# RoboticExplorationLab/TrajectoryOptimization.jl

Hardware: NVIDIA H100
Metric: ilqr_iterations_per_sec (higher is better)
Workload: dtype f64

## Files before the change

### profiles/linesearch_ab.py

```python
#!/usr/bin/env python3
import argparse, json, os, subprocess, sys, tempfile

import numpy as np

ROOT = os.path.dirname(os.path.dirname(os.path.abspath(__file__)))
DEFAULT = os.path.join(ROOT, "trajectoryoptimization.jl_b200", "libtrajopt_b200.so")
VARIANT = os.path.join(ROOT, "trajectoryoptimization.jl_b200", "variants", "lib_fwd_loop.so")


def card():
    q = subprocess.run(["nvidia-smi", "--query-gpu=name,power.limit,clocks.max.sm", "--format=csv,noheader"], capture_output=True, text=True)
    return q.stdout.strip().splitlines()[0] if q.returncode == 0 and q.stdout.strip() else "unknown"


def bench(lib, workload, dump):
    env = dict(os.environ, LIBTRAJOPT_B200=lib)
    out = subprocess.run([sys.executable, os.path.join(ROOT, "bench.py"), "--gpus", "1", "--steps", "20", "--warmup", "3", "--workload", workload,
                          "--no-cpu-baseline", "--dump-outputs", dump], capture_output=True, text=True, env=env, cwd=ROOT)
    line = [l for l in out.stdout.splitlines() if l.startswith("{")]
    if out.returncode or not line:
        raise SystemExit(f"bench.py failed on {lib}:\n{out.stderr[-2000:]}")
    d = json.loads(line[-1])
    ph = d["roofline"]["phase_ms"]
    return dict(step=d["ms_per_step"], F=ph["forward"], L=ph["ladder"], C1E1=ph["cost_expansion"] + ph["expand"],
                E2C2=ph["late_expansion"], R=ph["backward"], phases=ph)


def main():
    ap = argparse.ArgumentParser()
    ap.add_argument("--reps", type=int, default=3)
    ap.add_argument("--workload", default="quadrotor")
    ap.add_argument("--out", default=None)
    ap.add_argument("--lib", action="append", default=[], metavar="NAME=PATH", help="further libraries to alternate with the two")
    args = ap.parse_args()
    tmp = tempfile.mkdtemp(prefix="linesearch_ab_")
    variant = VARIANT
    if not os.path.exists(variant):
        subprocess.run(["bash", os.path.join(ROOT, "profiles", "scripts", "build_variant.sh"), "fwd_loop", "forward.cu", "-DTO_FWD_COMPACT=0"],
                       check=True, env=dict(os.environ, VARIANT_DIR=tmp), stdout=subprocess.DEVNULL)
        variant = os.path.join(tmp, "lib_fwd_loop.so")
    print(f"card: {card()}  workload: {args.workload}", flush=True)
    libs = {"rollout_fast (-DTO_FWD_COMPACT=0)": variant, "rollout_compact (default)": DEFAULT}
    libs.update(dict(kv.split("=", 1) for kv in args.lib))
    runs = {name: [] for name in libs}
    dumps = []
    for r in range(args.reps):
        for name, lib in libs.items():
            d = os.path.join(tmp, f"dump_{len(dumps)}")
            res = bench(lib, args.workload, d)
            runs[name].append(res); dumps.append((name, d))
            print(f"  {name:36s} step {res['step']:.4f}  F {res['F']:.4f}  L {res['L']:.4f}  C1+E1 {res['C1E1']:.4f}  "
                  f"E2/C2 {res['E2C2']:.4f}  R {res['R']:.4f}", flush=True)
    ref_name, ref = dumps[0]
    identical = True
    for name, d in dumps[1:]:
        for f in sorted(os.listdir(ref)):
            a, b = np.load(os.path.join(ref, f)), np.load(os.path.join(d, f))
            if a.shape != b.shape or not np.array_equal(a.view(np.uint8), b.view(np.uint8)):
                identical = False
                print(f"  DUMP DIFFERS: {f} of {name} against {ref_name}")
    print(f"dumps bit-identical across all {len(dumps)} runs: {identical}")
    for name, rs in runs.items():
        rng = lambda k: f"{min(x[k] for x in rs):.3f}-{max(x[k] for x in rs):.3f}"
        print(f"{name:36s} step {rng('step')}  F {rng('F')}  L {rng('L')}  C1+E1 {rng('C1E1')}  E2/C2 {rng('E2C2')}  R {rng('R')}")
    fa, fb = runs["rollout_fast (-DTO_FWD_COMPACT=0)"], runs["rollout_compact (default)"]
    print(f"every default run faster than every variant run: {max(x['step'] for x in fb) < min(x['step'] for x in fa)}")
    if args.out:
        with open(args.out, "w") as fh:
            json.dump(dict(card=card(), runs=runs, identical=identical), fh, indent=1)
    sys.exit(0 if identical else 1)


if __name__ == "__main__":
    main()
```

### trajectoryoptimization.jl_b200/csrc/capi.cu

```cuda
#include <cmath>
#include <cstdio>
#include <cstring>
#include <string>
#include <vector>

#include "../../include/trajopt_b200.h"
#include "frag_layout.cuh"
#include "kernels.h"

namespace {

std::string g_create_error;

struct Scratch {
    void* ptr = nullptr;
    size_t bytes = 0;
};

}

struct to_handle {
    DevProblem P{};
    int device = 0;
    cudaStream_t stream = nullptr;
// ... 559 lines not shown
        P.max_cons_knot = std::max(P.max_cons_knot, nk);
    }
    {
        bool cls = N >= 2 && P.all_diag_cost && P.all_diag_con;
        for (int k = 1; k < N - 1; k++) if (h->h_cost_index[k] != h->h_cost_index[0]) cls = false;
        int nbox = 0, ngc = 0;
        for (const auto& c : h->h_cons) {
            if (c.kind == CON_BOUND) {
                bool ubox = c.first == 1 && c.last == N - 1 && c.p == 2 * m;
                for (int j = 0; j < n + m; j++) if ((c.row_max[j] >= 0) != (j >= n) || (c.row_min[j] >= 0) != (j >= n)) ubox = false;
                cls = cls && ubox; nbox++;
            } else if (c.kind == CON_GOAL) {
                cls = cls && c.first == N && c.last == N; ngc++;
            } else cls = false;
        }
        P.fwd_compact = (cls && nbox <= 1 && ngc <= 1) ? 1 : 0;
    }
    h->h_mu.assign(s->ncon, P.opt.penalty_initial);
    h->h_dt.assign(s->dt, s->dt + (N - 1));
    h->h_dyn = dyn_tab; h->h_dyn_index = dyn_idx;

    int rc = TO_OK;
    double* d_dt = nullptr; int* d_ci = nullptr;
    P.strideX = (size_t)B * N * n; P.strideU = (size_t)B * (N - 1) * m;
#define ALLOC(ptr, count) if (!rc) rc = dalloc(h, &(ptr), (size_t)(count))
    ALLOC(d_dt, N - 1); ALLOC(d_ci, N);
    DevDyn* d_dyn = nullptr; int* d_dyni = nullptr;
    if (!h->h_dyn.empty()) { ALLOC(d_dyn, h->h_dyn.size()); ALLOC(d_dyni, N - 1); }
    ALLOC(h->d_costs, s->ncost); ALLOC(h->d_cons, std::max(1, s->ncon)); ALLOC(h->d_mu, std::max(1, s->ncon));
    ALLOC(P.x0, (size_t)B * n); ALLOC(P.X, TO_NBUF * P.strideX); ALLOC(P.U, TO_NBUF * P.strideU); ALLOC(P.cur, B);
    ALLOC(P.AB, (size_t)B * (N - 1) * n * P.ldab); ALLOC(P.K, (size_t)B * (N - 1) * P.ne * m); ALLOC(P.d, (size_t)B * (N - 1) * m);
    if (P.dense_riccati) {
        const size_t nme = P.ne + m;
        ALLOC(P.ABe, (size_t)B * (N - 1) * P.ne * nme); ALLOC(P.EG, (size_t)B * N * nme); ALLOC(P.EH, (size_t)B * N * nme * nme);
        if (P.compact) ALLOC(P.EC, (size_t)B * N * TO_EC_LEN);
        if (P.frag) ALLOC(P.REC, (size_t)B * N * TO_REC_LEN);
    }
    ALLOC(P.lambda, (size_t)B * std::max(1, P.lambda_len));
    ALLOC(P.rho, B); ALLOC(P.drho, B); ALLOC(P.dV, 2 * (size_t)B); ALLOC(P.J, B); ALLOC(P.Jc, B); ALLOC(P.alpha, B);
    ALLOC(P.bp_status, B); ALLOC(P.ls_iters, B); ALLOC(P.accepted, B); ALLOC(P.acc1, B);
    if (P.frag) { ALLOC(P.late_list, B); ALLOC(P.late_count, 1); }
    ALLOC(h->d_stageX, P.strideX); ALLOC(h->d_stageU, P.strideU); ALLOC(h->d_viol, B); ALLOC(h->d_merit2, 2);
    ALLOC(h->d_work, 1); ALLOC(h->d_err, 1);
    {
        SolveDev& S = h->solve;
        ALLOC(S.state, B); ALLOC(S.status, B); ALLOC(S.iter, B); ALLOC(S.outer, B); ALLOC(S.inner, B); ALLOC(S.dj_zero, B);
        ALLOC(S.J_prev, B); ALLOC(S.dJ, B); ALLOC(S.grad, B); ALLOC(S.cmax, B); ALLOC(S.n_active, 1);
    }
    if (P.frag) { ALLOC(h->d_fragq, frag_queue_ints(B)); ALLOC(h->d_fragpool, frag_pool_doubles(B, N)); ALLOC(h->d_fragerr, 1); ALLOC(h->d_exptab, 1); }
#undef ALLOC
    if (rc) return bail(rc);
    P.exptab = h->d_exptab;
    P.dyn = d_dyn; P.dyn_index = d_dyni;
    P.dt = d_dt; P.cost_index = d_ci; P.costs = h->d_costs; P.cons = h->d_cons; P.mu = h->d_mu; P.viol = h->d_viol;
    cudaStream_t st = h->stream;
    bool okc = true;
    okc &= cudaMemcpyAsync(d_dt, h->h_dt.data(), sizeof(double) * (N - 1), cudaMemcpyHostToDevice, st) == cudaSuccess;
    okc &= cudaMemcpyAsync(d_ci, h->h_cost_index.data(), sizeof(int) * N, cudaMemcpyHostToDevice, st) == cudaSuccess;
    if (d_dyn) {
        okc &= cudaMemcpyAsync(d_dyn, h->h_dyn.data(), sizeof(DevDyn) * h->h_dyn.size(), cudaMemcpyHostToDevice, st) == cudaSuccess;
        okc &= cudaMemcpyAsync(d_dyni, h->h_dyn_index.data(), sizeof(int) * (N - 1), cudaMemcpyHostToDevice, st) == cudaSuccess;
    }
    okc &= cudaMemsetAsync(P.x0, 0, sizeof(double) * B * n, st) == cudaSuccess;
    okc &= cudaMemsetAsync(P.X, 0xFF, sizeof(double) * TO_NBUF * P.strideX, st) == cudaSuccess;
    okc &= cudaMemsetAsync(P.U, 0, sizeof(double) * TO_NBUF * P.strideU, st) == cudaSuccess;
// ... 123 lines not shown
        if (upper) upper[i] = up;
    }
    return TO_OK;
}

int to_set_initial_state(to_handle* h, const double* x0) {
    JOIN(h);
    if (!h || !x0) return TO_EINVAL;
    CU(h, cudaMemcpyAsync(h->P.x0, x0, sizeof(double) * (size_t)h->P.B * h->P.n, cudaMemcpyHostToDevice, h->stream));
    h->J_valid = false;
    return TO_OK;
}
int to_set_controls(to_handle* h, const double* U) {
    JOIN(h);
    if (!h || !U) return TO_EINVAL;
    CU(h, cudaMemcpyAsync(h->d_stageU, U, sizeof(double) * h->P.strideU, cudaMemcpyHostToDevice, h->stream));
    CU(h, launch_scatter_traj(h->P, nullptr, h->d_stageU, h->stream)); h->launches++;
    h->J_valid = false; h->expanded = false; h->backward_done = false;
    return TO_OK;
}
int to_set_states(to_handle* h, const double* X) {
    JOIN(h);
    if (!h || !X) return TO_EINVAL;
    CU(h, cudaMemcpyAsync(h->d_stageX, X, sizeof(double) * h->P.strideX, cudaMemcpyHostToDevice, h->stream));
    CU(h, launch_scatter_traj(h->P, h->d_stageX, nullptr, h->stream)); h->launches++;
    h->J_valid = false; h->expanded = false; h->backward_done = false;
    return TO_OK;
}
int to_get_states(to_handle* h, double* X) {
    JOIN(h);
    if (!h || !X) return TO_EINVAL;
    CU(h, launch_gather_traj(h->P, h->d_stageX, nullptr, h->stream)); h->launches++;
    CU(h, cudaMemcpyAsync(X, h->d_stageX, sizeof(double) * h->P.strideX, cudaMemcpyDeviceToHost, h->stream));
    CU(h, cudaStreamSynchronize(h->stream));
    return TO_OK;
}
int to_get_controls(to_handle* h, double* U) {
    JOIN(h);
    if (!h || !U) return TO_EINVAL;
    CU(h, launch_gather_traj(h->P, nullptr, h->d_stageU, h->stream)); h->launches++;
    CU(h, cudaMemcpyAsync(U, h->d_stageU, sizeof(double) * h->P.strideU, cudaMemcpyDeviceToHost, h->stream));
    CU(h, cudaStreamSynchronize(h->stream));
    return TO_OK;
}
int to_get_times(to_handle* h, double* t) {
    JOIN(h);
    if (!h || !t) return TO_EINVAL;
    t[0] = h->t0;
    for (int k = 1; k < h->P.N; k++) t[k] = t[k - 1] + h->h_dt[k - 1];
    return TO_OK;
}
int to_set_initial_time(to_handle* h, double t0, double* tf_out) {
    JOIN(h);
    if (!h) return TO_EINVAL;
    h->t0 = t0;
    if (tf_out) { double t = t0; for (double d : h->h_dt) t += d; *tf_out = t; }
// ... 855 lines not shown
```

### trajectoryoptimization.jl_b200/csrc/common.cuh

```cuda
#pragma once
#include <cuda_runtime.h>
#include <cstdlib>
#include <stdint.h>

#define TO_MAXN 16
#define TO_MAXM 8
#define TO_MAXNM (TO_MAXN + TO_MAXM)
#define TO_MAXCON 8
#define TO_MAXP 32
#define TO_MAXPV (2 * TO_MAXNM)
#define TO_CON_A 256
#define TO_EXPR_LEN 128
#define TO_EXPR_CONST 64
#define TO_EC_LEN 40
#define TO_NBUF 9

enum { MODEL_DOUBLE_INTEGRATOR = 0, MODEL_CARTPOLE = 1, MODEL_QUADROTOR = 2, MODEL_ACROBOT = 3, MODEL_EXPR = 4 };
enum { CONE_ZERO = 0, CONE_NEGATIVE_ORTHANT = 1, CONE_SECOND_ORDER = 2, CONE_IDENTITY = 3, CONE_POSITIVE_ORTHANT = 4 };
enum { CON_GOAL = 0, CON_BOUND = 1, CON_LINEAR = 2, CON_CIRCLE = 3, CON_SPHERE = 4, CON_NORM = 5, CON_COLLISION = 6, CON_QUATVEC = 7, CON_EXPR = 8 };

struct DevCost {
    int diag, terminal, zeroH, pad;
    double c;
    double Qd[TO_MAXN], Rd[TO_MAXM];
// ... 88 lines not shown
    double* K;
    double* d;
    double* lambda;
    double* rho;
    double* drho;
    double* dV;
    double* J;
    double* Jc;
    double* viol;
    double* alpha;
    int* bp_status;
    int* ls_iters;
    int* accepted;
    int* acc1;
    int* late_list;
    int* late_count;
    size_t strideX, strideU;
    const int* active;
    const double* qr;
    int fwd_compact;
    const double* mparams;
    const double* cdata;
    int ncdata;
};
#define TO_NPARAM 16

enum { SOLVE_ACTIVE = 0, SOLVE_WAITING = 1, SOLVE_DONE = 2 };
__host__ __device__ inline bool retired(const DevProblem& P, int b) { return P.active != nullptr && P.active[b] != SOLVE_ACTIVE; }

__host__ __device__ inline bool inst_forward(const DevProblem& P) { return P.qr || P.mparams || P.cdata; }
__host__ __device__ inline bool inst_backward(const DevProblem& P) { return P.qr || P.cdata; }
__host__ __device__ inline bool inst_dynamics(const DevProblem& P) { return P.mparams; }

template <bool INST>
__host__ __device__ __forceinline__ const double* inst_q(const DevProblem& P, int b, int cid) {
    if constexpr (INST) { if (P.qr) return P.qr + ((size_t)b * P.ncost + cid) * (P.n + P.m); }
    return P.costs[cid].q;
}
template <bool INST>
__host__ __device__ __forceinline__ const double* inst_r(const DevProblem& P, int b, int cid) {
    if constexpr (INST) { if (P.qr) return P.qr + ((size_t)b * P.ncost + cid) * (P.n + P.m) + P.n; }
    return P.costs[cid].r;
}
template <bool INST>
__device__ __forceinline__ double model_param(const DevProblem& P, int b, int i) {
    if constexpr (INST) { if (P.mparams) return P.mparams[(size_t)b * TO_NPARAM + i]; }
// ... 5 lines not shown
    return shared;
}
struct ConData { const double *a, *b, *c3, *rad; double val; };
template <bool INST>
__device__ __forceinline__ ConData con_data(const DevProblem& P, int b, int ci) {
    const DevCon& con = P.cons[ci];
    ConData d{con.a, con.b, con.c3, con.rad, con.val};
    if constexpr (INST) {
        if (P.cdata && con.cdoff >= 0) {
            const double* row = con_row<true>(P, b, ci, nullptr);
            switch (con.kind) {
                case CON_GOAL: d.a = row; break;
                case CON_BOUND: d.a = row; d.b = row + P.n + P.m; break;
                case CON_LINEAR: d.b = row; break;
                case CON_CIRCLE: d.a = row; d.b = row + con.p; d.rad = row + 2 * con.p; break;
                case CON_SPHERE: d.a = row; d.b = row + con.p; d.c3 = row + 2 * con.p; d.rad = row + 3 * con.p; break;
                case CON_NORM: case CON_COLLISION: d.val = row[0]; break;
            }
        }
    }
    return d;
}

__host__ __device__ inline const double* traj_X(const DevProblem& P, int buf, int b) { return P.X + buf * P.strideX + (size_t)b * P.N * P.n; }
__host__ __device__ inline const double* traj_U(const DevProblem& P, int buf, int b) { return P.U + buf * P.strideU + (size_t)b * (P.N - 1) * P.m; }
__host__ __device__ inline double* traj_Xw(const DevProblem& P, int buf, int b) { return P.X + buf * P.strideX + (size_t)b * P.N * P.n; }
__host__ __device__ inline double* traj_Uw(const DevProblem& P, int buf, int b) { return P.U + buf * P.strideU + (size_t)b * (P.N - 1) * P.m; }

#define TO_MAXDEV 64
inline int current_device_slot() { int d = 0; cudaGetDevice(&d); return (d >= 0 && d < TO_MAXDEV) ? d : 0; }

__host__ __device__ inline void reg_increase(const DevOptions& o, double& rho, double& drho) {
    drho = fmax(drho * o.bp_reg_increase_factor, o.bp_reg_increase_factor);
    rho = fmax(rho * drho, o.bp_reg_min);
}
__host__ __device__ inline void reg_decrease(const DevOptions& o, double& rho, double& drho) {
    drho = fmin(drho / o.bp_reg_increase_factor, 1.0 / o.bp_reg_increase_factor);
    rho = rho * drho * ((rho * drho > o.bp_reg_min) ? 1.0 : 0.0);
}
```

### trajectoryoptimization.jl_b200/csrc/forward.cu

```cuda
#include <cstdlib>
#include <type_traits>
#include "costcon.cuh"
#include "kernels.h"
#include "models.cuh"

namespace {

constexpr int FWD_MAX_COST = 4;
constexpr int FWD_MAX_N = 512;
constexpr int FWD_THREADS = 32;

struct FwdCon {
    int kind, first, last, p, offset;
    unsigned mask_max, mask_min;
    int ubox;
    double mu, inv2mu;
    int row_max[TO_MAXNM], row_min[TO_MAXNM];
    double a[TO_MAXNM], b[TO_MAXNM];
};
struct FwdCost {
    double Qd[TO_MAXN], Rd[TO_MAXM], q[TO_MAXN], r[TO_MAXM], c;
};
struct alignas(16) FwdTab {
    int ncon, ncost_cached, pad0, pad1;
    FwdCon con[TO_MAXCON];
    FwdCost cost[FWD_MAX_COST];
    double dt[FWD_MAX_N];
// ... 80 lines not shown
                unsigned mx = 0;
                for (int j = 0; j < TO_MAXNM; j++) if (k.row_max[j] >= 0) mx |= 1u << j;
                f.mask_max = mx;
            }
            for (int j = t; j < TO_MAXNM; j += T) { f.row_max[j] = k.row_max[j]; f.a[j] = k.a[j]; }
        }
    }
    for (int k = t; k < P.N - 1; k += T) tab.dt[k] = P.dt[k];
    __syncthreads();
}

__device__ __forceinline__ void cp_async8(double* smem_dst, const double* gsrc) {
    asm volatile("cp.async.ca.shared.global [%0], [%1], 8;" ::"r"((uint32_t)__cvta_generic_to_shared(smem_dst)), "l"(gsrc) : "memory");
}
__device__ __forceinline__ void cp_async16(double* smem_dst, const double* gsrc) {
    asm volatile("cp.async.cg.shared.global [%0], [%1], 16;" ::"r"((uint32_t)__cvta_generic_to_shared(smem_dst)), "l"(gsrc) : "memory");
}
__device__ __forceinline__ void cp_async_commit() { asm volatile("cp.async.commit_group;" ::: "memory"); }
#ifndef TO_FWD_STAGES
#define TO_FWD_STAGES 2
#endif
constexpr int FWD_STAGES = TO_FWD_STAGES;
constexpr int FWD_OKNOTS = 4;
template <int NPEND> __device__ __forceinline__ void cp_async_wait() { asm volatile("cp.async.wait_group %0;" ::"n"(NPEND) : "memory"); }

template <int n, int m, int IPB, int NE = n>
struct Stage {
    static constexpr int KSLOTS = NE * m;
    static constexpr bool K16 = (KSLOTS % 2) == 0;
    static constexpr int OFF_D = KSLOTS, OFF_U = OFF_D + m, OFF_X = OFF_U + m, OFF_L = OFF_X + n;
    static constexpr int LAM_SLOTS = 2 * (n + m);
    static constexpr int NSLOT = OFF_L + LAM_SLOTS;
    static constexpr int DOUBLES = NSLOT * IPB;
    __device__ static __forceinline__ int kidx(int e, int g) { return K16 ? ((e >> 1) * IPB + g) * 2 + (e & 1) : e * IPB + g; }
    __device__ static __forceinline__ int sidx(int slot, int g) { return slot * IPB + g; }
};

template <int n, int m, int IPB, int G, int NE>
__device__ __forceinline__ void prefetch_operands(double* base, int g, int l, int k, const double* Kg, const double* dg, const double* X,
                                                  const double* U, int N) {
    using S = Stage<n, m, IPB, NE>;
    if (k < N - 1) {
        const double* Kk = Kg + (size_t)k * NE * m;
        if (S::K16) {
#pragma unroll
            for (int c = 0; c < (S::KSLOTS / 2 + G - 1) / G; c++) {
// ... 186 lines not shown
                slot += c.p;
            }
        }
        if (!last) {
            rk4_step<MODEL, double>(model_params<MODEL, INST>(P, prm, k), x, u, tab.dt[k], xn);
#pragma unroll
            for (int i = 0; i < n; i++) { x[i] = xn[i]; if (!(fabs(xn[i]) <= P.opt.max_state_value)) ok = false; }
        }
    }
    cp_async_wait<0>();
    return J;
}

template <int MODEL, int IPB, int G, bool LIE, bool INST>
__device__ __forceinline__ double rollout_compact(const DevProblem& P, const FwdCompactTab& tab, double* stage, double* ost, const double* prm,
                                                  const double2* gbox, int b, int g, int l, unsigned gmask, double alpha, int cbuf, bool& ok,
                                                  double& viol) {
    constexpr int n = ModelDims<MODEL>::n, m = ModelDims<MODEL>::m, NE = LIE ? n - 1 : n;
    using S = Stage<n, m, IPB, NE>;
    const int N = P.N, buf = P.cur[b];
    const double* X = traj_X(P, buf, b);
    const double* U = traj_U(P, buf, b);
    double* Xc = traj_Xw(P, cbuf, b);
    const double* Kg = P.K + (size_t)b * (N - 1) * NE * m;
    const double* dg = P.d + (size_t)b * (N - 1) * m;
    const double* lam_b = P.lambda + (size_t)b * P.lambda_len;
    constexpr int OX = FWD_OKNOTS * n, OL = FWD_OKNOTS * (n + m);
    double* myx = ost + l * OL;
    double* myu = myx + OX;
    const double* cq = INST ? inst_q<true>(P, b, tab.cid) : nullptr;
    const double* cr = INST ? inst_r<true>(P, b, tab.cid) : nullptr;
    const bool box = tab.box_p != 0;
    double x[n], u[m];
    double J = 0.0;
    ok = true; viol = 0.0;
#pragma unroll
    for (int i = 0; i < n; i++) x[i] = P.x0[(size_t)b * n + i];
    constexpr int D = FWD_STAGES - 1;
    auto prefetch = [&](double* base, int k) {
        prefetch_operands<n, m, IPB, G, NE>(base, g, l, k, Kg, dg, X, U, N);
        const bool stg = k < N - 1;
        const int cnt = stg ? tab.box_p : tab.goal_p;
        const double* src = lam_b + (stg ? tab.box_off + k * tab.box_p : tab.goal_off);
        for (int i = l; i < cnt; i += G) cp_async8(base + S::sidx(S::OFF_L + i, g), src + i);
    };
#pragma unroll
    for (int j = 0; j < D; j++) {
        if (j < N) prefetch(stage + j * S::DOUBLES, j);
        cp_async_commit();
    }
    int sb = 0, sp = D;
    auto next_stage = [&](int k) -> const double* {
        __syncwarp(gmask);
        if (k + D < N) prefetch(stage + sp * S::DOUBLES, k + D);
        cp_async_commit();
        cp_async_wait<D>();
        __syncwarp(gmask);
        const double* st = stage + sb * S::DOUBLES;
        sb = (sb + 1 == FWD_STAGES) ? 0 : sb + 1; sp = (sp + 1 == FWD_STAGES) ? 0 : sp + 1;
        return st;
    };
    auto knot = [&](int k, double* x) {
        const double* st = next_stage(k);
#pragma unroll
        for (int a = 0; a < m; a++) u[a] = fma(alpha, st[S::sidx(S::OFF_D + a, g)], st[S::sidx(S::OFF_U + a, g)]);
        double dxe[NE];
// ... 4 lines not shown
            state_diff(true, n, 3, x, xr, dxe);
        } else {
#pragma unroll
            for (int i = 0; i < n; i++) dxe[i] = x[i] - st[S::sidx(S::OFF_X + i, g)];
        }
#pragma unroll
        for (int i = 0; i < NE; i++) {
            const double dx = dxe[i];
            if (S::K16 && (m % 2 == 0)) {
#pragma unroll
                for (int a = 0; a < m; a += 2) {
                    const double2 kv = *reinterpret_cast<const double2*>(&st[S::kidx(i * m + a, g)]);
                    u[a] = fma(kv.x, dx, u[a]);
                    u[a + 1] = fma(kv.y, dx, u[a + 1]);
                }
            } else {
#pragma unroll
                for (int a = 0; a < m; a++) u[a] = fma(st[S::kidx(i * m + a, g)], dx, u[a]);
            }
        }
#pragma unroll
        for (int a = 0; a < m; a++) if (!(fabs(u[a]) <= P.opt.max_control_value)) ok = false;
        const int kk = k % FWD_OKNOTS;
#pragma unroll
        for (int i = 0; i < n; i++) myx[kk * n + i] = x[i];
#pragma unroll
        for (int a = 0; a < m; a++) myu[kk * m + a] = u[a];
        if (kk == FWD_OKNOTS - 1 || k == N - 2) {
            __syncwarp(gmask);
            const int k0 = k - kk, nx = (kk + 1) * n, nu = (kk + 1) * m;
            for (int j = 0; j < G; j++) {
                const int cb = (buf + 1 + j) % TO_NBUF;
                double* xd = traj_Xw(P, cb, b) + (size_t)k0 * n;
                double* ud = traj_Uw(P, cb, b) + (size_t)k0 * m;
                const double* xs = ost + j * OL;
                for (int e = l; e < nx; e += G) xd[e] = xs[e];
                for (int e = l; e < nu; e += G) ud[e] = xs[OX + e];
            }
        }
        {
            double a2 = 0.0, l1 = 0.0;
#pragma unroll
            for (int i = 0; i < n; i++) { const double2 c = tab.sx[i]; a2 = fma(c.x * x[i], x[i], a2); l1 = fma(INST ? cq[i] : c.y, x[i], l1); }
#pragma unroll
            for (int i = 0; i < m; i++) { const double2 c = tab.su[i]; a2 = fma(c.x * u[i], u[i], a2); l1 = fma(INST ? cr[i] : c.y, u[i], l1); }
            J += fma(0.5, a2, l1) + tab.sc;
        }
        if (box) {
            const double mu = tab.mu;
            double a = 0.0, l2 = 0.0;
#pragma unroll
            for (int i = 0; i < m; i++) {
                const double lu = st[S::sidx(S::OFF_L + i, g)], ll = st[S::sidx(S::OFF_L + m + i, g)];
                const double2 bx = INST ? gbox[i] : tab.box[i];
                const double cu = u[i] - bx.x, cl = bx.y - u[i];
                const double vu = fma(-mu, cu, lu), vl = fma(-mu, cl, ll);
                const double pu = vu < 0.0 ? vu : 0.0, pl = vl < 0.0 ? vl : 0.0;
                a = fma(pu, pu, a); a = fma(pl, pl, a); l2 = fma(lu, lu, l2); l2 = fma(ll, ll, l2);
                const double t = cu > cl ? cu : cl;
                viol = t > viol ? t : viol;
// ... 150 lines not shown
    if (work) {
        const int trial = trial0 + l;
        const double alpha = ldexp(1.0, -trial);
        const int cbuf = (P.cur[b] + 1 + l) % TO_NBUF;
        bool ok = false;
        double J, viol = 0.0;
        double* prm = nullptr;
        double2* gbox = nullptr;
        if constexpr (INST) {
            prm = reinterpret_cast<double*>(fwd_smem + ls_smem_bytes<MODEL, G, PATH, LANES, LIE>()) + g * TO_NPARAM;
            if (l == 0) stage_model_params<INST>(P, b, prm);
            if constexpr (PATH == FWD_COMPACT) {
                gbox = reinterpret_cast<double2*>(reinterpret_cast<double*>(fwd_smem + ls_smem_bytes<MODEL, G, PATH, LANES, LIE>()) + IPB * TO_NPARAM) + g * TO_MAXM;
                if (tab->box_p != 0)
                    for (int ci = 0; ci < P.ncon; ci++)
                        if (P.cons[ci].kind == CON_BOUND) {
                            const ConData cd = con_data<true>(P, b, ci);
                            for (int i = l; i < m; i += G) gbox[i] = make_double2(cd.a[n + i], cd.b[n + i]);
                        }
            }
            __syncwarp(gmask);
        }
        if constexpr (PATH == FWD_COMPACT) {
            double* ost = stage + FWD_STAGES * S::DOUBLES + (size_t)g * G * FWD_OKNOTS * (n + m);
            J = rollout_compact<MODEL, IPB, G, LIE, INST>(P, *tab, stage, ost, prm, gbox, b, g, l, gmask, alpha, cbuf, ok, viol);
        }
        else if (FAST) J = rollout_fast<MODEL, IPB, G, LIE, INST>(P, *tab, stage, prm, b, g, l, gmask, alpha, cbuf, ok, viol);
        else J = rollout_generic<MODEL, LIE, INST>(P, prm, b, alpha, cbuf, ok, viol);
        const bool good = (trial <= P.opt.ls_iters) && ls_accept(P, J, P.J[b], alpha, P.dV[2 * b], P.dV[2 * b + 1], ok);
        const unsigned votes = __ballot_sync(gmask, good) & gmask;
        if (votes) {
            const int win = __ffs(votes) - 1 - g * G;
            if (l == win) {
                P.cur[b] = cbuf; P.J[b] = J; P.viol[b] = viol; P.alpha[b] = alpha; P.ls_iters[b] = trial + 1; P.accepted[b] = 1;
            }
            accepted = true;
        }
    }
    if (l == 0 && first_pass) {
        P.acc1[b] = accepted ? 1 : 0;
        if (!accepted && P.late_list) P.late_list[atomicAdd(P.late_count, 1)] = b;
    }
    if (l == 0 && !accepted) {
        if (first_pass) P.accepted[b] = 0;
        if (status < 0) { P.alpha[b] = 0.0; P.ls_iters[b] = 0; }
        else if (final_pass) {
            double rho = P.rho[b], drho = P.drho[b];
            reg_increase(P.opt, rho, drho);
            rho += P.opt.bp_reg_fp;
            P.rho[b] = rho; P.drho[b] = drho;
            P.alpha[b] = 0.0; P.ls_iters[b] = P.opt.ls_iters + 1;
        }
    }
    (void)sizeof(S);
}

template <int MODEL, int G, bool FAST, int LANES, bool LIE, bool INST>
__global__ void __launch_bounds__(FWD_THREADS) k_linesearch(const DevProblem P, int trial0, int first_pass, int final_pass) {
    linesearch_pass<MODEL, G, FAST ? FWD_FAST : FWD_GENERIC, LANES, LIE, INST>(P, trial0, first_pass, final_pass);
}

template <int MODEL, int G, int LANES, bool LIE, bool INST>
__global__ void __launch_bounds__(FWD_THREADS) k_linesearch_compact(const DevProblem P, int trial0, int first_pass, int final_pass) {
    linesearch_pass<MODEL, G, FWD_COMPACT, LANES, LIE, INST>(P, trial0, first_pass, final_pass);
}

template <int MODEL, int G, int PATH, int LANES, bool LIE = false, bool INST = false>
cudaError_t launch_pass_l(const DevProblem& P, int trial0, int first_pass, int final_pass, cudaStream_t s) {
    constexpr int IPB = LANES / G;
    const int blocks = (P.B + IPB - 1) / IPB;
    static_assert(ls_smem_bytes<MODEL, G, PATH, LANES, LIE>() % 16 == 0, "the parameter rows and the staged boxes (double2) follow the tables");
    const size_t smem = ls_smem_bytes<MODEL, G, PATH, LANES, LIE>() + (INST ? (size_t)IPB * TO_NPARAM * sizeof(double) : 0)
                      + (INST && PATH == FWD_COMPACT ? (size_t)IPB * TO_MAXM * sizeof(double2) : 0);
    auto kern = [] {
        if constexpr (PATH == FWD_COMPACT) return k_linesearch_compact<MODEL, G, LANES, LIE, INST>;
        else return k_linesearch<MODEL, G, PATH == FWD_FAST, LANES, LIE, INST>;
// ... 70 lines not shown
```

### trajectoryoptimization.jl_b200/csrc/riccati.cu

```cuda
#include <cstddef>

#include "costcon.cuh"
#include "kernels.h"

#ifndef TO_RICCATI_STAGES
#define TO_RICCATI_STAGES 2
#endif
#ifndef TO_RICCATI_MINB
#define TO_RICCATI_MINB 16
#endif

#ifdef TO_RICCATI_MAXREG
#define TO_RICCATI_BOUNDS(MINB) __maxnreg__(TO_RICCATI_MAXREG)
#else
#define TO_RICCATI_BOUNDS(MINB) __launch_bounds__(32, MINB)
#endif

namespace {

__host__ __device__ constexpr int even_up(int v) { return (v + 1) & ~1; }
constexpr int MAXT = 3;

__device__ __forceinline__ double2 lds128(const double* p) { return *reinterpret_cast<const double2*>(p); }
__device__ __forceinline__ void sts128(double* p, double a, double b) { *reinterpret_cast<double2*>(p) = make_double2(a, b); }

__device__ __forceinline__ uint32_t smem_u32(const void* p) { return (uint32_t)__cvta_generic_to_shared(p); }
__device__ __forceinline__ void mbar_init(uint64_t* bar, uint32_t count) {
    asm volatile("mbarrier.init.shared::cta.b64 [%0], %1;" ::"r"(smem_u32(bar)), "r"(count));
}
__device__ __forceinline__ void mbar_expect_tx(uint64_t* bar, uint32_t bytes) {
    asm volatile("mbarrier.arrive.expect_tx.shared::cta.b64 _, [%0], %1;" ::"r"(smem_u32(bar)), "r"(bytes) : "memory");
}
__device__ __forceinline__ void mbar_wait(uint64_t* bar, uint32_t parity) {
    asm volatile(
        "{\n\t.reg .pred p;\n\t"
        "WAIT_LOOP:\n\t"
        "mbarrier.try_wait.parity.shared::cta.b64 p, [%0], %1;\n\t"
        "@p bra DONE;\n\t"
        "bra WAIT_LOOP;\n\t"
        "DONE:\n\t}" ::"r"(smem_u32(bar)), "r"(parity) : "memory");
}
__device__ __forceinline__ void bulk_g2s(void* dst, const void* src, uint32_t bytes, uint64_t* bar) {
    asm volatile("cp.async.bulk.shared::cluster.global.mbarrier::complete_tx::bytes [%0], [%1], %2, [%3];" ::"r"(smem_u32(dst)),
                 "l"(src), "r"(bytes), "r"(smem_u32(bar))
                 : "memory");
}

__device__ __forceinline__ double ldg_pinned(const double* p) {
    double v;
    asm volatile("ld.global.nc.f64 %0, [%1];" : "=d"(v) : "l"(p));
    return v;
}

__device__ __forceinline__ int ldg_pinned(const int* p) {
    int v;
    asm volatile("ld.global.nc.s32 %0, [%1];" : "=r"(v) : "l"(p));
    return v;
}

__device__ __forceinline__ double rcp_pivot(double x) {
    double y;
    asm("rcp.approx.ftz.f64 %0, %1;" : "=d"(y) : "d"(x));
    double e = fma(-x, y, 1.0);
    y = fma(y, e, y);
    e = fma(-x, y, 1.0);
    return fma(y, e, y);
}

__device__ __forceinline__ void fma2x2(double (&acc)[4], const double2& a, const double2& b) {
// ... 881 lines not shown
```

### trajectoryoptimization.jl_b200/csrc/riccati_frag.cu

```cuda
#include "costcon.cuh"
#include "frag_layout.cuh"
#include "kernels.h"

#ifndef TO_FRAG_STAGES
#define TO_FRAG_STAGES 2
#endif
#ifndef TO_FRAG_WARPS
#define TO_FRAG_WARPS 4
#endif
#ifndef TO_FRAG_ROUNDS
#define TO_FRAG_ROUNDS 2
#endif
#ifndef TO_FRAG_MINB
#define TO_FRAG_MINB 4
#endif
#ifndef TO_FRAG_PF
#define TO_FRAG_PF 0
#endif

namespace {

inline unsigned nblk(long long total, int threads) { return (unsigned)((total + threads - 1) / threads); }

__device__ __forceinline__ uint32_t smem_u32(const void* p) { return (uint32_t)__cvta_generic_to_shared(p); }
__device__ __forceinline__ void mbar_init(uint64_t* bar, uint32_t count) {
    asm volatile("mbarrier.init.shared::cta.b64 [%0], %1;" ::"r"(smem_u32(bar)), "r"(count));
}
__device__ __forceinline__ void mbar_expect_tx(uint64_t* bar, uint32_t bytes) {
    asm volatile("mbarrier.arrive.expect_tx.shared::cta.b64 _, [%0], %1;" ::"r"(smem_u32(bar)), "r"(bytes) : "memory");
}
__device__ __forceinline__ void mbar_wait(uint64_t* bar, uint32_t parity) {
    asm volatile(
        "{\n\t.reg .pred p;\n\t"
        "WAIT_LOOP:\n\t"
        "mbarrier.try_wait.parity.shared::cta.b64 p, [%0], %1;\n\t"
        "@p bra DONE;\n\t"
        "bra WAIT_LOOP;\n\t"
        "DONE:\n\t}" ::"r"(smem_u32(bar)), "r"(parity) : "memory");
}
__device__ __forceinline__ void bulk_g2s(void* dst, const void* src, uint32_t bytes, uint64_t* bar) {
    asm volatile("cp.async.bulk.shared::cluster.global.mbarrier::complete_tx::bytes [%0], [%1], %2, [%3];" ::"r"(smem_u32(dst)),
                 "l"(src), "r"(bytes), "r"(smem_u32(bar))
                 : "memory");
}
__device__ __forceinline__ void bulk_prefetch_l2(const void* src, uint32_t bytes) {
    asm volatile("cp.async.bulk.prefetch.L2.global [%0], %1;" ::"l"(src), "r"(bytes) : "memory");
}
__device__ __forceinline__ double2 lds128(const double* p) { return *reinterpret_cast<const double2*>(p); }
__device__ __forceinline__ void dmma(double& d0, double& d1, double a, double b) {
    asm volatile("mma.sync.aligned.m8n8k4.row.col.f64.f64.f64.f64 {%0,%1}, {%2}, {%3}, {%0,%1};" : "+d"(d0), "+d"(d1) : "d"(a), "d"(b));
}
__device__ __forceinline__ int ld_volatile_s32(const int* p) {
    int v;
    asm volatile("ld.volatile.global.s32 %0, [%1];" : "=r"(v) : "l"(p) : "memory");
    return v;
}
__device__ __forceinline__ void tile_transpose(double x0, double x1, int src, int odd_row, double& y0, double& y1) {
    const double a0 = __shfl_sync(0xffffffffu, x0, src), a1 = __shfl_sync(0xffffffffu, x1, src);
    const double b0 = __shfl_sync(0xffffffffu, x0, src + 4), b1 = __shfl_sync(0xffffffffu, x1, src + 4);
    y0 = odd_row ? a1 : a0;
    y1 = odd_row ? b1 : b0;
}
__device__ __forceinline__ double rcp_pos(double x) {
    double y;
    asm("rcp.approx.ftz.f64 %0, %1;" : "=d"(y) : "d"(x));
    double e = fma(-x, y, 1.0);
    y = fma(y, e, y);
    e = fma(-x, y, 1.0);
    return fma(y, e, y);
}
// ... 499 lines not shown
```

Baseline: 2.966 million.

## Store compact rollout trajectories with bulk async shared-to-global copies

The compact forward rollout now writes each lane's staged states and controls to global memory using cp.async.bulk shared-to-global copies, replacing the cooperative per-lane store loop across the group. To make those copies aligned, the per-trajectory X stride is padded to an even length (ldX), and staging-buffer reuse is guarded with bulk wait_group.read. Shared TMA helpers move into a common header, and debug knobs (NOSTORE/NOLOAD) plus the A/B script are generalised. The intent is to cut store instructions and the warp syncs in the rollout, at the cost of extra async bookkeeping and a padded X layout.

Result: faster. 2.997 million (median of 6 runs) (+1.0%).

```diff
diff --git a/profiles/linesearch_ab.py b/profiles/linesearch_ab.py
--- a/profiles/linesearch_ab.py
+++ b/profiles/linesearch_ab.py
@@ -1,11 +1,10 @@
 #!/usr/bin/env python3
-import argparse, json, os, subprocess, sys, tempfile
+import argparse, json, os, re, subprocess, sys, tempfile
 
 import numpy as np
 
 ROOT = os.path.dirname(os.path.dirname(os.path.abspath(__file__)))
 DEFAULT = os.path.join(ROOT, "trajectoryoptimization.jl_b200", "libtrajopt_b200.so")
-VARIANT = os.path.join(ROOT, "trajectoryoptimization.jl_b200", "variants", "lib_fwd_loop.so")
 
 
 def card():
@@ -31,24 +30,32 @@
     ap.add_argument("--reps", type=int, default=3)
     ap.add_argument("--workload", default="quadrotor")
     ap.add_argument("--out", default=None)
+    ap.add_argument("--flags", default="-DTO_FWD_BULK=0", help="the variant's build flags for forward.cu")
     ap.add_argument("--lib", action="append", default=[], metavar="NAME=PATH", help="further libraries to alternate with the two")
+    ap.add_argument("--timing-only", action="append", default=[], metavar="NAME=PATH", help="... left out of the bitwise comparison")
     args = ap.parse_args()
     tmp = tempfile.mkdtemp(prefix="linesearch_ab_")
-    variant = VARIANT
+    vname = "fwd_" + re.sub(r"[^a-z0-9]+", "", args.flags.lower().replace("-dto_fwd_", " ").replace("=", ""))
+    variant = os.path.join(ROOT, "trajectoryoptimization.jl_b200", "variants", f"lib_{vname}.so")
     if not os.path.exists(variant):
-        subprocess.run(["bash", os.path.join(ROOT, "profiles", "scripts", "build_variant.sh"), "fwd_loop", "forward.cu", "-DTO_FWD_COMPACT=0"],
+        subprocess.run(["bash", os.path.join(ROOT, "profiles", "scripts", "build_variant.sh"), vname, "forward.cu", args.flags],
                        check=True, env=dict(os.environ, VARIANT_DIR=tmp), stdout=subprocess.DEVNULL)
-        variant = os.path.join(tmp, "lib_fwd_loop.so")
+        variant = os.path.join(tmp, f"lib_{vname}.so")
     print(f"card: {card()}  workload: {args.workload}", flush=True)
-    libs = {"rollout_fast (-DTO_FWD_COMPACT=0)": variant, "rollout_compact (default)": DEFAULT}
+    vlabel, dlabel = f"variant ({args.flags})", "default"
+    libs = {vlabel: variant, dlabel: DEFAULT}
     libs.update(dict(kv.split("=", 1) for kv in args.lib))
+    timing_only = dict(kv.split("=", 1) for kv in args.timing_only)
+    libs.update(timing_only)
     runs = {name: [] for name in libs}
     dumps = []
     for r in range(args.reps):
         for name, lib in libs.items():
-            d = os.path.join(tmp, f"dump_{len(dumps)}")
+            d = os.path.join(tmp, f"dump_{r}_{len(dumps)}")
             res = bench(lib, args.workload, d)
-            runs[name].append(res); dumps.append((name, d))
+            runs[name].append(res)
+            if name not in timing_only:
+                dumps.append((name, d))
             print(f"  {name:36s} step {res['step']:.4f}  F {res['F']:.4f}  L {res['L']:.4f}  C1+E1 {res['C1E1']:.4f}  "
                   f"E2/C2 {res['E2C2']:.4f}  R {res['R']:.4f}", flush=True)
     ref_name, ref = dumps[0]
@@ -59,15 +66,15 @@
             if a.shape != b.shape or not np.array_equal(a.view(np.uint8), b.view(np.uint8)):
                 identical = False
                 print(f"  DUMP DIFFERS: {f} of {name} against {ref_name}")
-    print(f"dumps bit-identical across all {len(dumps)} runs: {identical}")
+    print(f"dumps bit-identical across all {len(dumps)} compared runs: {identical}")
     for name, rs in runs.items():
         rng = lambda k: f"{min(x[k] for x in rs):.3f}-{max(x[k] for x in rs):.3f}"
         print(f"{name:36s} step {rng('step')}  F {rng('F')}  L {rng('L')}  C1+E1 {rng('C1E1')}  E2/C2 {rng('E2C2')}  R {rng('R')}")
-    fa, fb = runs["rollout_fast (-DTO_FWD_COMPACT=0)"], runs["rollout_compact (default)"]
+    fa, fb = runs[vlabel], runs[dlabel]
     print(f"every default run faster than every variant run: {max(x['step'] for x in fb) < min(x['step'] for x in fa)}")
     if args.out:
         with open(args.out, "w") as fh:
-            json.dump(dict(card=card(), runs=runs, identical=identical), fh, indent=1)
+            json.dump(dict(card=card(), workload=args.workload, runs=runs, identical=identical), fh, indent=1)
     sys.exit(0 if identical else 1)
 
 
diff --git a/trajectoryoptimization.jl_b200/csrc/capi.cu b/trajectoryoptimization.jl_b200/csrc/capi.cu
--- a/trajectoryoptimization.jl_b200/csrc/capi.cu
+++ b/trajectoryoptimization.jl_b200/csrc/capi.cu
@@ -605,7 +605,9 @@
 
     int rc = TO_OK;
     double* d_dt = nullptr; int* d_ci = nullptr;
-    P.strideX = (size_t)B * N * n; P.strideU = (size_t)B * (N - 1) * m;
+    P.ldX = (N * n + 1) & ~1;
+    P.strideX = (size_t)B * P.ldX; P.strideU = (size_t)B * (N - 1) * m;
+    const size_t nX = (size_t)B * N * n;
 #define ALLOC(ptr, count) if (!rc) rc = dalloc(h, &(ptr), (size_t)(count))
     ALLOC(d_dt, N - 1); ALLOC(d_ci, N);
     DevDyn* d_dyn = nullptr; int* d_dyni = nullptr;
@@ -623,7 +625,7 @@
     ALLOC(P.rho, B); ALLOC(P.drho, B); ALLOC(P.dV, 2 * (size_t)B); ALLOC(P.J, B); ALLOC(P.Jc, B); ALLOC(P.alpha, B);
     ALLOC(P.bp_status, B); ALLOC(P.ls_iters, B); ALLOC(P.accepted, B); ALLOC(P.acc1, B);
     if (P.frag) { ALLOC(P.late_list, B); ALLOC(P.late_count, 1); }
-    ALLOC(h->d_stageX, P.strideX); ALLOC(h->d_stageU, P.strideU); ALLOC(h->d_viol, B); ALLOC(h->d_merit2, 2);
+    ALLOC(h->d_stageX, nX); ALLOC(h->d_stageU, P.strideU); ALLOC(h->d_viol, B); ALLOC(h->d_merit2, 2);
     ALLOC(h->d_work, 1); ALLOC(h->d_err, 1);
     {
         SolveDev& S = h->solve;
@@ -793,7 +795,7 @@
 int to_set_states(to_handle* h, const double* X) {
     JOIN(h);
     if (!h || !X) return TO_EINVAL;
-    CU(h, cudaMemcpyAsync(h->d_stageX, X, sizeof(double) * h->P.strideX, cudaMemcpyHostToDevice, h->stream));
+    CU(h, cudaMemcpyAsync(h->d_stageX, X, sizeof(double) * h->P.B * h->P.N * h->P.n, cudaMemcpyHostToDevice, h->stream));
     CU(h, launch_scatter_traj(h->P, h->d_stageX, nullptr, h->stream)); h->launches++;
     h->J_valid = false; h->expanded = false; h->backward_done = false;
     return TO_OK;
@@ -802,7 +804,7 @@
     JOIN(h);
     if (!h || !X) return TO_EINVAL;
     CU(h, launch_gather_traj(h->P, h->d_stageX, nullptr, h->stream)); h->launches++;
-    CU(h, cudaMemcpyAsync(X, h->d_stageX, sizeof(double) * h->P.strideX, cudaMemcpyDeviceToHost, h->stream));
+    CU(h, cudaMemcpyAsync(X, h->d_stageX, sizeof(double) * h->P.B * h->P.N * h->P.n, cudaMemcpyDeviceToHost, h->stream));
     CU(h, cudaStreamSynchronize(h->stream));
     return TO_OK;
 }
diff --git a/trajectoryoptimization.jl_b200/csrc/common.cuh b/trajectoryoptimization.jl_b200/csrc/common.cuh
--- a/trajectoryoptimization.jl_b200/csrc/common.cuh
+++ b/trajectoryoptimization.jl_b200/csrc/common.cuh
@@ -134,6 +134,7 @@
     const double* mparams;
     const double* cdata;
     int ncdata;
+    int ldX;
 };
 #define TO_NPARAM 16
 
@@ -185,9 +186,9 @@
     return d;
 }
 
-__host__ __device__ inline const double* traj_X(const DevProblem& P, int buf, int b) { return P.X + buf * P.strideX + (size_t)b * P.N * P.n; }
+__host__ __device__ inline const double* traj_X(const DevProblem& P, int buf, int b) { return P.X + buf * P.strideX + (size_t)b * P.ldX; }
 __host__ __device__ inline const double* traj_U(const DevProblem& P, int buf, int b) { return P.U + buf * P.strideU + (size_t)b * (P.N - 1) * P.m; }
-__host__ __device__ inline double* traj_Xw(const DevProblem& P, int buf, int b) { return P.X + buf * P.strideX + (size_t)b * P.N * P.n; }
+__host__ __device__ inline double* traj_Xw(const DevProblem& P, int buf, int b) { return P.X + buf * P.strideX + (size_t)b * P.ldX; }
 __host__ __device__ inline double* traj_Uw(const DevProblem& P, int buf, int b) { return P.U + buf * P.strideU + (size_t)b * (P.N - 1) * P.m; }
 
 #define TO_MAXDEV 64
diff --git a/trajectoryoptimization.jl_b200/csrc/forward.cu b/trajectoryoptimization.jl_b200/csrc/forward.cu
--- a/trajectoryoptimization.jl_b200/csrc/forward.cu
+++ b/trajectoryoptimization.jl_b200/csrc/forward.cu
@@ -3,6 +3,7 @@
 #include "costcon.cuh"
 #include "kernels.h"
 #include "models.cuh"
+#include "tma.cuh"
 
 namespace {
 
@@ -129,6 +130,16 @@
 #endif
 constexpr int FWD_STAGES = TO_FWD_STAGES;
 constexpr int FWD_OKNOTS = 4;
+#ifndef TO_FWD_BULK
+#define TO_FWD_BULK 1
+#endif
+#ifndef TO_FWD_NOSTORE
+#define TO_FWD_NOSTORE 0
+#endif
+#ifndef TO_FWD_NOLOAD
+#define TO_FWD_NOLOAD 0
+#endif
+template <int MODEL> __host__ __device__ constexpr bool fwd_bulk() { return TO_FWD_BULK && FWD_OKNOTS * ModelDims<MODEL>::n * sizeof(double) >= 256; }
 template <int NPEND> __device__ __forceinline__ void cp_async_wait() { asm volatile("cp.async.wait_group %0;" ::"n"(NPEND) : "memory"); }
 
 template <int n, int m, int IPB, int NE = n>
@@ -361,6 +372,7 @@
     const double* X = traj_X(P, buf, b);
     const double* U = traj_U(P, buf, b);
     double* Xc = traj_Xw(P, cbuf, b);
+    double* Uc = traj_Uw(P, cbuf, b);
     const double* Kg = P.K + (size_t)b * (N - 1) * NE * m;
     const double* dg = P.d + (size_t)b * (N - 1) * m;
     const double* lam_b = P.lambda + (size_t)b * P.lambda_len;
@@ -377,10 +389,11 @@
     for (int i = 0; i < n; i++) x[i] = P.x0[(size_t)b * n + i];
     constexpr int D = FWD_STAGES - 1;
     auto prefetch = [&](double* base, int k) {
-        prefetch_operands<n, m, IPB, G, NE>(base, g, l, k, Kg, dg, X, U, N);
         const bool stg = k < N - 1;
+        const int ko = (TO_FWD_NOLOAD && stg) ? 0 : k;
+        prefetch_operands<n, m, IPB, G, NE>(base, g, l, ko, Kg, dg, X, U, N);
         const int cnt = stg ? tab.box_p : tab.goal_p;
-        const double* src = lam_b + (stg ? tab.box_off + k * tab.box_p : tab.goal_off);
+        const double* src = lam_b + (stg ? tab.box_off + ko * tab.box_p : tab.goal_off);
         for (int i = l; i < cnt; i += G) cp_async8(base + S::sidx(S::OFF_L + i, g), src + i);
     };
 #pragma unroll
@@ -431,20 +444,40 @@
 #pragma unroll
         for (int a = 0; a < m; a++) if (!(fabs(u[a]) <= P.opt.max_control_value)) ok = false;
         const int kk = k % FWD_OKNOTS;
+        if constexpr (fwd_bulk<MODEL>()) { if (kk == 0) bulk_wait_read<0>(); }
 #pragma unroll
         for (int i = 0; i < n; i++) myx[kk * n + i] = x[i];
 #pragma unroll
         for (int a = 0; a < m; a++) myu[kk * m + a] = u[a];
-        if (kk == FWD_OKNOTS - 1 || k == N - 2) {
-            __syncwarp(gmask);
+        if (!TO_FWD_NOSTORE && (kk == FWD_OKNOTS - 1 || k == N - 2)) {
             const int k0 = k - kk, nx = (kk + 1) * n, nu = (kk + 1) * m;
-            for (int j = 0; j < G; j++) {
-                const int cb = (buf + 1 + j) % TO_NBUF;
-                double* xd = traj_Xw(P, cb, b) + (size_t)k0 * n;
-                double* ud = traj_Uw(P, cb, b) + (size_t)k0 * m;
-                const double* xs = ost + j * OL;
-                for (int e = l; e < nx; e += G) xd[e] = xs[e];
-                for (int e = l; e < nu; e += G) ud[e] = xs[OX + e];
+            if constexpr (fwd_bulk<MODEL>()) {
+                const bool bx = (nx & 1) == 0, bu = ((nu | (N - 1) * m) & 1) == 0;
+                if (bx || bu) {
+                    fence_proxy_async_smem();
+                    if (bx) bulk_s2g(Xc + (size_t)k0 * n, myx, nx * sizeof(double));
+                    if (bu) bulk_s2g(Uc + (size_t)k0 * m, myu, nu * sizeof(double));
+                    bulk_commit();
+                }
+                if (!(bx && bu)) {
+                    __syncwarp(gmask);
+                    for (int j = 0; j < G; j++) {
+                        const int cb = (buf + 1 + j) % TO_NBUF;
+                        const double* xs = ost + j * OL;
+                        if (!bx) { double* xd = traj_Xw(P, cb, b) + (size_t)k0 * n; for (int e = l; e < nx; e += G) xd[e] = xs[e]; }
+                        if (!bu) { double* ud = traj_Uw(P, cb, b) + (size_t)k0 * m; for (int e = l; e < nu; e += G) ud[e] = xs[OX + e]; }
+                    }
+                }
+            } else {
+                __syncwarp(gmask);
+                for (int j = 0; j < G; j++) {
+                    const int cb = (buf + 1 + j) % TO_NBUF;
+                    double* xd = traj_Xw(P, cb, b) + (size_t)k0 * n;
+                    double* ud = traj_Uw(P, cb, b) + (size_t)k0 * m;
+                    const double* xs = ost + j * OL;
+                    for (int e = l; e < nx; e += G) xd[e] = xs[e];
+                    for (int e = l; e < nu; e += G) ud[e] = xs[OX + e];
+                }
             }
         }
         {
@@ -641,6 +674,7 @@
             __syncwarp(gmask);
         }
         if constexpr (PATH == FWD_COMPACT) {
+            static_assert(sizeof(Tab) % 16 == 0 && S::DOUBLES % 2 == 0, "each lane's output staging starts on 16 bytes (the source of its bulk copies)");
             double* ost = stage + FWD_STAGES * S::DOUBLES + (size_t)g * G * FWD_OKNOTS * (n + m);
             J = rollout_compact<MODEL, IPB, G, LIE, INST>(P, *tab, stage, ost, prm, gbox, b, g, l, gmask, alpha, cbuf, ok, viol);
         }
@@ -671,6 +705,7 @@
             P.alpha[b] = 0.0; P.ls_iters[b] = P.opt.ls_iters + 1;
         }
     }
+    if constexpr (PATH == FWD_COMPACT && fwd_bulk<MODEL>()) { if (work) bulk_wait<0>(); }
     (void)sizeof(S);
 }
 
diff --git a/trajectoryoptimization.jl_b200/csrc/riccati.cu b/trajectoryoptimization.jl_b200/csrc/riccati.cu
--- a/trajectoryoptimization.jl_b200/csrc/riccati.cu
+++ b/trajectoryoptimization.jl_b200/csrc/riccati.cu
@@ -2,6 +2,7 @@
 
 #include "costcon.cuh"
 #include "kernels.h"
+#include "tma.cuh"
 
 #ifndef TO_RICCATI_STAGES
 #define TO_RICCATI_STAGES 2
@@ -23,28 +24,6 @@
 
 __device__ __forceinline__ double2 lds128(const double* p) { return *reinterpret_cast<const double2*>(p); }
 __device__ __forceinline__ void sts128(double* p, double a, double b) { *reinterpret_cast<double2*>(p) = make_double2(a, b); }
-
-__device__ __forceinline__ uint32_t smem_u32(const void* p) { return (uint32_t)__cvta_generic_to_shared(p); }
-__device__ __forceinline__ void mbar_init(uint64_t* bar, uint32_t count) {
-    asm volatile("mbarrier.init.shared::cta.b64 [%0], %1;" ::"r"(smem_u32(bar)), "r"(count));
-}
-__device__ __forceinline__ void mbar_expect_tx(uint64_t* bar, uint32_t bytes) {
-    asm volatile("mbarrier.arrive.expect_tx.shared::cta.b64 _, [%0], %1;" ::"r"(smem_u32(bar)), "r"(bytes) : "memory");
-}
-__device__ __forceinline__ void mbar_wait(uint64_t* bar, uint32_t parity) {
-    asm volatile(
-        "{\n\t.reg .pred p;\n\t"
-        "WAIT_LOOP:\n\t"
-        "mbarrier.try_wait.parity.shared::cta.b64 p, [%0], %1;\n\t"
-        "@p bra DONE;\n\t"
-        "bra WAIT_LOOP;\n\t"
-        "DONE:\n\t}" ::"r"(smem_u32(bar)), "r"(parity) : "memory");
-}
-__device__ __forceinline__ void bulk_g2s(void* dst, const void* src, uint32_t bytes, uint64_t* bar) {
-    asm volatile("cp.async.bulk.shared::cluster.global.mbarrier::complete_tx::bytes [%0], [%1], %2, [%3];" ::"r"(smem_u32(dst)),
-                 "l"(src), "r"(bytes), "r"(smem_u32(bar))
-                 : "memory");
-}
 
 __device__ __forceinline__ double ldg_pinned(const double* p) {
     double v;
diff --git a/trajectoryoptimization.jl_b200/csrc/riccati_frag.cu b/trajectoryoptimization.jl_b200/csrc/riccati_frag.cu
--- a/trajectoryoptimization.jl_b200/csrc/riccati_frag.cu
+++ b/trajectoryoptimization.jl_b200/csrc/riccati_frag.cu
@@ -1,6 +1,7 @@
 #include "costcon.cuh"
 #include "frag_layout.cuh"
 #include "kernels.h"
+#include "tma.cuh"
 
 #ifndef TO_FRAG_STAGES
 #define TO_FRAG_STAGES 2
@@ -22,30 +23,6 @@
 
 inline unsigned nblk(long long total, int threads) { return (unsigned)((total + threads - 1) / threads); }
 
-__device__ __forceinline__ uint32_t smem_u32(const void* p) { return (uint32_t)__cvta_generic_to_shared(p); }
-__device__ __forceinline__ void mbar_init(uint64_t* bar, uint32_t count) {
-    asm volatile("mbarrier.init.shared::cta.b64 [%0], %1;" ::"r"(smem_u32(bar)), "r"(count));
-}
-__device__ __forceinline__ void mbar_expect_tx(uint64_t* bar, uint32_t bytes) {
-    asm volatile("mbarrier.arrive.expect_tx.shared::cta.b64 _, [%0], %1;" ::"r"(smem_u32(bar)), "r"(bytes) : "memory");
-}
-__device__ __forceinline__ void mbar_wait(uint64_t* bar, uint32_t parity) {
-    asm volatile(
-        "{\n\t.reg .pred p;\n\t"
-        "WAIT_LOOP:\n\t"
-        "mbarrier.try_wait.parity.shared::cta.b64 p, [%0], %1;\n\t"
-        "@p bra DONE;\n\t"
-        "bra WAIT_LOOP;\n\t"
-        "DONE:\n\t}" ::"r"(smem_u32(bar)), "r"(parity) : "memory");
-}
-__device__ __forceinline__ void bulk_g2s(void* dst, const void* src, uint32_t bytes, uint64_t* bar) {
-    asm volatile("cp.async.bulk.shared::cluster.global.mbarrier::complete_tx::bytes [%0], [%1], %2, [%3];" ::"r"(smem_u32(dst)),
-                 "l"(src), "r"(bytes), "r"(smem_u32(bar))
-                 : "memory");
-}
-__device__ __forceinline__ void bulk_prefetch_l2(const void* src, uint32_t bytes) {
-    asm volatile("cp.async.bulk.prefetch.L2.global [%0], %1;" ::"l"(src), "r"(bytes) : "memory");
-}
 __device__ __forceinline__ double2 lds128(const double* p) { return *reinterpret_cast<const double2*>(p); }
 __device__ __forceinline__ void dmma(double& d0, double& d1, double a, double b) {
     asm volatile("mma.sync.aligned.m8n8k4.row.col.f64.f64.f64.f64 {%0,%1}, {%2}, {%3}, {%0,%1};" : "+d"(d0), "+d"(d1) : "d"(a), "d"(b));
diff --git a/trajectoryoptimization.jl_b200/csrc/tma.cuh b/trajectoryoptimization.jl_b200/csrc/tma.cuh
--- /dev/null
+++ b/trajectoryoptimization.jl_b200/csrc/tma.cuh
@@ -0,0 +1,39 @@
+#pragma once
+#include <stdint.h>
+
+namespace {
+
+__device__ __forceinline__ uint32_t smem_u32(const void* p) { return (uint32_t)__cvta_generic_to_shared(p); }
+__device__ __forceinline__ void mbar_init(uint64_t* bar, uint32_t count) {
+    asm volatile("mbarrier.init.shared::cta.b64 [%0], %1;" ::"r"(smem_u32(bar)), "r"(count));
+}
+__device__ __forceinline__ void mbar_expect_tx(uint64_t* bar, uint32_t bytes) {
+    asm volatile("mbarrier.arrive.expect_tx.shared::cta.b64 _, [%0], %1;" ::"r"(smem_u32(bar)), "r"(bytes) : "memory");
+}
+__device__ __forceinline__ void mbar_wait(uint64_t* bar, uint32_t parity) {
+    asm volatile(
+        "{\n\t.reg .pred p;\n\t"
+        "WAIT_LOOP:\n\t"
+        "mbarrier.try_wait.parity.shared::cta.b64 p, [%0], %1;\n\t"
+        "@p bra DONE;\n\t"
+        "bra WAIT_LOOP;\n\t"
+        "DONE:\n\t}" ::"r"(smem_u32(bar)), "r"(parity) : "memory");
+}
+__device__ __forceinline__ void bulk_g2s(void* dst, const void* src, uint32_t bytes, uint64_t* bar) {
+    asm volatile("cp.async.bulk.shared::cluster.global.mbarrier::complete_tx::bytes [%0], [%1], %2, [%3];" ::"r"(smem_u32(dst)),
+                 "l"(src), "r"(bytes), "r"(smem_u32(bar))
+                 : "memory");
+}
+__device__ __forceinline__ void bulk_prefetch_l2(const void* src, uint32_t bytes) {
+    asm volatile("cp.async.bulk.prefetch.L2.global [%0], %1;" ::"l"(src), "r"(bytes) : "memory");
+}
+
+__device__ __forceinline__ void fence_proxy_async_smem() { asm volatile("fence.proxy.async.shared::cta;" ::: "memory"); }
+__device__ __forceinline__ void bulk_s2g(void* dst, const void* src, uint32_t bytes) {
+    asm volatile("cp.async.bulk.global.shared::cta.bulk_group [%0], [%1], %2;" ::"l"(dst), "r"(smem_u32(src)), "r"(bytes) : "memory");
+}
+__device__ __forceinline__ void bulk_commit() { asm volatile("cp.async.bulk.commit_group;" ::: "memory"); }
+template <int NPEND> __device__ __forceinline__ void bulk_wait_read() { asm volatile("cp.async.bulk.wait_group.read %0;" ::"n"(NPEND) : "memory"); }
+template <int NPEND> __device__ __forceinline__ void bulk_wait() { asm volatile("cp.async.bulk.wait_group %0;" ::"n"(NPEND) : "memory"); }
+
+}
```
